# divortio/divortio-lz4

Measured on AMD Instinct MI355X. Metric: LZ4 compress+decompress GB/s on 4 MiB independent blocks; % of HBM peak, higher is better.
Workload: dtype u8; 1 GPU; raw block decompress, 4096 x 4 MiB independent blocks per GPU (tiles216), device-resident (BASELINE.json configs[1]); blocks_per_gpu=4096, block_bytes=4194304, generator=tiles216, parallelism=blocks sharded x1

## Files before the change

divortio-lz4_amd/csrc/lz4mi_decompress.hip:

```cpp
#include "../../include/lz4mi.h"
#include "lz4mi_common.h"
#include "lz4mi_decompress.h"
#include "lz4mi_launch.h"

#ifndef LZ4MI_LL_ADAPT
#define LZ4MI_LL_ADAPT 127
#endif
#ifndef LZ4MI_ORDER
#define LZ4MI_ORDER 1
#endif
#ifndef LZ4MI_ABLATE
#define LZ4MI_ABLATE 0
#endif

#ifndef LZ4MI_TIMELINE
#define LZ4MI_TIMELINE 0
#endif

#ifndef LZ4MI_PROFILE
#define LZ4MI_PROFILE 0
#endif

namespace lz4mi {

// ... 639 lines not shown
            }
            P += lane_of(incl, kWave - 1);
            R += (uint32_t)__popcll(bal);
        }
        __syncthreads();
        PieceGen g{L, bm, P, 0u, -1, lane};
        while (64u * g.t < P) {
            LSlot sl[kPieceBatch];
            uint4 v[kPieceBatch];
            g.template fill<kPieceBatch>(sl);
#pragma unroll
            for (int j = 0; j < kPieceBatch; ++j) {
                const u32x4_t t = *(const u32x4_t*)(c.dst + (sl[j].w ? sl[j].a : 0));
                v[j] = make_uint4(t.x, t.y, t.z, t.w);
            }
            lane_store<kPieceBatch>(c, S, sl, v);
        }
        __syncthreads();
    }
}

__device__ __forceinline__ void lane_slow_run(const Ctx& c, const DecShared& S, const Run& R) {
    const int np = run_pieces(R.n);
    for (int p = 0; p < np; ++p) {
        const Piece P = plan_piece(R, p);
        if (P.mode == 4) {
            bytes_piece(c, P.y, P.a, P.b, P.w, P.period);
            continue;
        }
        const uint4 A = load16<R_HIST>(c, S, P.a);
        uint4 v = A;
        if (P.mode == 2) v = pick4(A, load16<R_HIST>(c, S, P.b), P.k);
        else if (P.mode == 3) v = expand_period(A, P.k, P.period);
        store_w(c.dst + P.y, v, P.w);
    }
}

__device__ __forceinline__ void periodic_run(const Ctx& c, const DecShared& S, int lane, const Run& R, PatBuf B) {
    const int32_t per = R.period;
    const uint8_t* src = c.dst + R.src;
    const int32_t W = B.bytes - 48;
    const int32_t dl = R.n - 16;
    for (int32_t s0 = 0; s0 < per; s0 += W) {
        const int32_t e0 = per - s0 <= W ? per : s0 + W;
        __syncthreads();
        for (int k = lane; 16 * k < e0 - s0 + 20; k += kWave) {
            const int32_t q = s0 + 16 * k;
            uint4 v;
            if (q + 16 <= per) {
                v = load16<R_HIST>(c, S, R.src + q);
            } else {
                unsigned __int128 x = 0;
#pragma unroll 1
                for (int j = 0; j < 16; ++j) x |= (unsigned __int128)src[(q + j) % per] << (8 * j);
                __builtin_memcpy(&v, &x, 16);
            }
            B.w[4 * k] = v.x;
            B.w[4 * k + 1] = v.y;
            B.w[4 * k + 2] = v.z;
            B.w[4 * k + 3] = v.w;
        }
        __syncthreads();
        const int32_t a0 = (int32_t)((0u - (uint32_t)(uintptr_t)(c.dst + R.y)) & 15u);
        if (lane == 0 && a0) {
            const int32_t ph = 0 - s0;
            if ((uint32_t)ph < (uint32_t)(e0 - s0)) out16(c.dst + R.y, stage16(B.w, ph));
        }
        const int32_t np = (R.n - a0 + 15) >> 4;
        const int32_t step = (16 * kWave) % per;
        int32_t r = (a0 + 16 * lane) % per;
#pragma unroll 2
        for (int32_t p = lane; p < np; p += kWave) {
            const int32_t d0 = a0 + 16 * p;
            const bool last = d0 > dl;
            const int32_t d = last ? dl : d0;
            const int32_t ph = (last ? d % per : r) - s0;
            if ((uint32_t)ph < (uint32_t)(e0 - s0) && LZ4MI_ABLATE != 4) {
                out16(c.dst + R.y + d, stage16(B.w, ph));
            }
            r += step;
            if (r >= per) r -= per;
        }
    }
    __syncthreads();
}


__device__ __forceinline__ void long_literals(uint8_t* dst, const uint8_t* src, int32_t n, int lane) {
    const int32_t np = (n + 15) >> 4;
    auto at = [&](int32_t p) { return 16 * p < n - 16 ? 16 * p : n - 16; };
#if LZ4MI_LL_ADAPT
    const unsigned int* lat = &g_lat_active[32 * xcc_id()];
#endif
    for (int32_t p0 = lane; p0 < np; p0 += kWave * 4) {
#if LZ4MI_LL_ADAPT
        const uint32_t busy = __hip_atomic_load(lat, __ATOMIC_RELAXED, __HIP_MEMORY_SCOPE_AGENT);
#endif
        const int32_t d0 = at(p0), d1 = at(p0 + kWave), d2 = at(p0 + 2 * kWave), d3 = at(p0 + 3 * kWave);
        uint4 v0, v1, v2, v3;
        v0 = ld16_nt(src + d0);
        v1 = ld16_nt(src + d1);
        v2 = ld16_nt(src + d2);
        v3 = ld16_nt(src + d3);
        st16_nt(dst + d0, v0);
        st16_nt(dst + d1, v1);
        st16_nt(dst + d2, v2);
        st16_nt(dst + d3, v3);
#if LZ4MI_LL_ADAPT
        if (busy) __builtin_amdgcn_s_sleep(LZ4MI_LL_ADAPT);
#endif
    }
}

__device__ __forceinline__ void wave_run(const Ctx& c, DecShared& S, int lane, const Run& R, PatBuf B) {
    if (R.kind == R_NONE || R.n <= 0) return;
    const bool in_buf = R.kind == R_HIST || (R.kind == R_BYTES && c.out_off + R.src >= 0);
    if (in_buf && R.period && R.n > kPeriodBulk &&
        B.bytes > 0 && (R.period + 48 <= B.bytes || (R.n >= 4 * R.period && B.bytes >= 1024))) {
        periodic_run(c, S, lane, R, B);
        return;
    }
    const int np = run_pieces(R.n);
    if (R.kind == R_BYTES) {
        for (int p = lane; p < np; p += kWave) {
            const Piece P = plan_piece(R, p);
            bytes_piece(c, P.y, P.a, P.b, P.w, P.period);
        }
        return;
    }
    if (R.period) {
        WaveGen<kWaveB2> g{R, np, 0, lane};
        pipe<R_HIST, true, kWaveB2>(c, S, g);
        return;
    }
    WaveGen<kWaveB> g{R, np, 0, lane};
    if (R.kind == R_LDS) pipe<R_LDS, false, kWaveB>(c, S, g);
    else if (R.kind == R_COMP && R.n >= kLongLit) long_literals(c.dst + R.y, c.blk + R.src, R.n, lane);
    else if (R.kind == R_COMP) pipe<R_COMP, false, kWaveB>(c, S, g);
    else pipe<R_HIST, false, kWaveB>(c, S, g);
}

__device__ __forceinline__ void short_literals(const Ctx& c, int32_t y, int32_t n, const uint4& v) {
    if (LZ4MI_ABLATE == 4) return;
    uint8_t* d = c.dst + y;
    uint64_t lo = v.x | ((uint64_t)v.y << 32);
    const uint64_t hi = v.z | ((uint64_t)v.w << 32);
    int32_t o = 0;
    if (n & 8) { __builtin_memcpy(d, &lo, 8); lo = hi; o = 8; }
    if (n & 4) { const uint32_t t = (uint32_t)lo; __builtin_memcpy(d + o, &t, 4); lo >>= 32; o += 4; }
    if (n & 2) { const uint16_t t = (uint16_t)lo; __builtin_memcpy(d + o, &t, 2); lo >>= 16; o += 2; }
    if (n & 1) d[o] = (uint8_t)lo;
}

__device__ __forceinline__ void lane_literals(const Ctx& c, const DecShared& S, const Run& L) {
    const int32_t n = L.kind == R_NONE ? 0 : L.n;
    const int np = n >= 16 ? (n + 15) >> 4 : 0;
    for (int q = 0; __ballot(q < np) != 0; q += 2) {
        const int32_t d0 = 16 * q < n - 16 ? 16 * q : n - 16, d1 = 16 * (q + 1) < n - 16 ? 16 * (q + 1) : n - 16;
        const uint4 v0 = stage16(S.stage, L.src + d0);
        const uint4 v1 = stage16(S.stage, L.src + d1);
        if (LZ4MI_ABLATE == 4) continue;
        if (q < np) out16(c.dst + L.y + d0, v0);
        if (q + 1 < np) out16(c.dst + L.y + d1, v1);
    }
    if (__ballot(n > 0 && n < 16)) {
        if (n > 0 && n < 16) short_literals(c, L.y, n, stage16(S.stage, L.src));
    }
}

__device__ __forceinline__ int64_t wave_varint(const Ctx& c, int lane, int64_t& q) {
    int64_t sum = 0;
    for (;;) {
        int64_t p = q + 16 * lane;
        int first = 16;
        uint32_t lastb = 0;
        for (int j = 0; j < 16; ++j) {
            int64_t r = p + j;
            uint32_t b = (r < c.in_len) ? c.blk[r] : 0u;
            if (b != 255u && first == 16) { first = j; lastb = b; }
        }
        uint64_t mask = __ballot(first < 16);
        if (mask) {
            int fl = __builtin_ctzll(mask);
            int fi = lane_of(first, fl);
            uint32_t fb = lane_of(lastb, fl);
            int64_t cnt = (int64_t)fl * 16 + fi;
            sum += 255 * cnt + fb;
            q += cnt + 1;
            return sum;
        }
        sum += 255 * 16 * kWave;
        q += 16 * kWave;
    }
}

__device__ __forceinline__ uint32_t seq_error(const Ctx& c, int64_t out_start, int64_t lit, int64_t ll, uint32_t off,
                                              int64_t ml) {
    if (out_start + ll > c.cap) return 1;
    if (lit + ll > c.in_len) return 2;
    if (ml == 0) return 0;
    if (off == 0) return 3;
    int64_t ms_abs = c.out_off + out_start + ll;
    if ((int64_t)off > ms_abs + c.dict_len) return 4;
    if (c.isolate && (int64_t)off > out_start + ll) return 5;
    return 0;
}

__device__ __forceinline__ int32_t err_status(uint32_t e) { return e == 5 ? -9 : -(int32_t)e; }
template <bool XP>
__device__ __forceinline__ uint32_t seq_err(const Ctx& c, bool rel, int64_t out_start, int64_t lit, int64_t ll,
                                            uint32_t off, int64_t ml) {
    if (XP && rel) {
        if (lit + ll > c.in_len) return 2;
        if (ml == 0) return 0;
        return off == 0 ? 3u : 0u;
    }
    return seq_error(c, out_start, lit, ll, off, ml);
}

__device__ __forceinline__ uint32_t f1_changes(const Ctx& c, int32_t ms, int32_t off, int32_t ml) {
    if (ml == 0 || ml >= 8 || off < 8 || c.out_off + ms - off < 0) return 0;
    const int32_t p0 = ms + ml - 8;
    if (p0 - off < 0) return c.isolate ? 2u : 1u;
    for (int32_t p = p0; p < ms && p < c.cap; ++p)
        if (hist_u8(c.dst + p) != hist_u8(c.dst + p - off)) return 1;
    return 0;
}

__device__ __noinline__ void f1_fixup(const Ctx c, const DecShared& S, int lane, uint32_t nseq, bool cut, int64_t cut_ms,
                         int32_t coff, int32_t cml) {
    int64_t lo = INT64_MAX;
    const uint32_t n = nseq + (cut ? 1u : 0u);
    for (uint32_t k = 0; k < n; ++k) {
        int64_t ms;
        int32_t off, ml;
        if (k < nseq) {
            const SeqInfo q = seq_info(S, k);
            ms = (int64_t)q.out + q.ll;
            off = q.off;
            ml = q.ml;
        } else {
            ms = cut_ms;
            off = coff;
            ml = cml;
        }
        if (ml == 0) continue;
        const bool internal = c.out_off + ms - off >= 0;
        if (ms - off + ml > lo) {
            if (internal) {
                for (int32_t t = lane; t < ml; t += kWave) {
                    const int64_t d = ms + t;
                    const int64_t s = ms - off + (off < ml ? t % off : t);
                    const uint32_t v = hist_u8(c.dst + s);
                    if (d < c.cap) c.dst[d] = (uint8_t)v;
                }
            } else if (lane == 0) {
                for (int32_t t = 0; t < ml; ++t) {
                    const uint32_t v = hist_byte(c, ms - off + t);
                    if (ms + t < c.cap) c.dst[ms + t] = (uint8_t)v;
                }
            }
            wait_vmem();
        }
        if (internal && off >= 8 && ml < 8) {
            const int64_t p = ms + ml - 8 + lane;
            const bool mine = lane < 8 - ml && c.out_off + p >= 0 && p < c.cap;
            const uint32_t v = mine ? (c.out_off + p - off >= 0 ? hist_u8(c.dst + p - off) : 0u) : 0u;
            if (mine) c.dst[p] = (uint8_t)v;
            const int64_t p0 = ms + ml - 8;
            if (p0 < lo) lo = p0;
            wait_vmem();
        }
    }
}

__device__ __forceinline__ void stored_block(const DecArgs& a, const Ctx& c, uint32_t b, uint32_t out_cap, int lane) {
    int32_t status = 0;
    const int32_t n = c.in_len;
    if ((uint32_t)n > out_cap) {
        status = LZ4MI_ERR_RANGE_STATUS;
    } else if (n >= 16) {
        long_literals(c.dst, c.blk, n, lane);
    } else if (lane < n) {
        c.dst[lane] = c.blk[lane];
    }
    if (lane == 0) {
        a.status[b] = status;
        a.out_len[b] = status ? 0u : (uint32_t)n;
    }
}

struct XState {
    bool on = false;
    uint4* xs = nullptr;
    SegRec* xr = nullptr;
    uint32_t seg_lo = 0, seg_hi = 0;
    bool started = false, done = false, fail = false;
    uint32_t G = 0, X = 0, nx = 0, olen = 0, err = 0xFFFFFFFFu, entry = 0;
    int64_t OG = 0;
    int pass = 0, restart = 0;
};

template <bool LK>
__device__ __forceinline__ bool x_enter(const DecArgs& a, Ctx& c, XState& x, int lane, uint32_t wblk, uint32_t sg,
                                        uint32_t nseg, uint32_t out_cap) {
    x.on = LK || ((uint32_t)c.in_len <= a.x_in_max && out_cap <= a.x_out_max &&
                  (uint64_t)out_cap < (uint64_t)c.in_len * kXRatioMax &&
                  !(a.x_flat1 && (uint64_t)c.in_len * 16 >= (uint64_t)out_cap * 15));
    if (!x.on) return a.xphase == 0 && sg == wblk % nseg;
    const SegGeom G = seg_geom((uint32_t)c.in_len);
    if (sg >= G.S) return false;
    x.seg_lo = sg * G.L;
    x.seg_hi = sg + 1 == G.S ? (uint32_t)c.in_len : min((uint32_t)c.in_len, x.seg_lo + G.L);
    x.xs = a.xseq + (size_t)wblk * a.xseq_stride + (size_t)sg * G.stride;
    x.xr = a.xrec + (size_t)wblk * nseg + sg;
    SegRec* const xr = x.xr;
    if (a.xphase == 2) {
        const uint32_t from = uniform(xr->from);
        if (from == kNoBase) return false;
        x.pass = 2;
        x.entry = from;
    }
    if (a.xphase == 1) {
        const uint32_t sstar = a.xfirst[wblk];
        if (sg < sstar) return false;
        uint32_t fp = 0;
        if (sg == sstar) {
            fp = xr[-1].exit;
        } else {
            if (lane == 0) {
                const uint32_t* f = &xr[-1].fin;
                while ((fp = __hip_atomic_load(f, __ATOMIC_ACQUIRE, __HIP_MEMORY_SCOPE_AGENT)) == 0u)
                    __builtin_amdgcn_s_sleep(8);
            }
            fp = lane_of(fp, 0) - 1u;
        }
        uint32_t fin = 0;
        bool reparse = false;
        if (fp == kFinErr) {
            fin = kFinErr;
            if (lane == 0) { xr->cnt = 0; xr->olen = 0; xr->err = 0xFFFFFFFFu; }
        } else if (fp >= x.seg_hi) {
            fin = fp;
            if (lane == 0) { xr->entry = xr->exit = fp; xr->cnt = 0; xr->olen = 0; xr->err = 0xFFFFFFFFu; }
        } else if (sg != sstar && !xr->fail && xr->entry == fp) {
            fin = xr->err != 0xFFFFFFFFu ? kFinErr : xr->exit;
        } else {
            reparse = true;
        }
        if (!reparse) {
            if (lane == 0) __hip_atomic_store(&xr->fin, fin + 1u, __ATOMIC_RELEASE, __HIP_MEMORY_SCOPE_AGENT);
            return false;
        }
        x.pass = 1;
        x.entry = fp;
    }
    c.ip = x.pass ? (int32_t)x.entry
                  : (x.seg_lo >= (uint32_t)c.in_len ? c.in_len : (int32_t)(x.seg_lo - min(x.seg_lo, kSegWarm)));
    return true;
}

__device__ __forceinline__ void stage_loads(const Ctx& c, int64_t at, int lane, uint4& p0, uint4& p1) {
    p0 = stage_piece(c, at + 16 * opaque(lane));
    if (lane < kStageWords / 4 - kWave) p1 = stage_piece(c, at + 16 * (kWave + opaque(lane)));
}
__device__ __forceinline__ void stage_write(DecShared& S, int lane, const uint4& p0, const uint4& p1) {
    __builtin_memcpy((uint8_t*)S.stage + 16 * lane, &p0, 16);
    if (lane < kStageWords / 4 - kWave) __builtin_memcpy((uint8_t*)S.stage + 16 * (kWave + lane), &p1, 16);
}

struct Prefetch {
    uint4 pf0 = make_uint4(0, 0, 0, 0), pf1 = make_uint4(0, 0, 0, 0);
    int64_t pf_at = -1;
    bool have_pf = false;
};
__device__ __forceinline__ void prefetch(const Ctx& c, Prefetch& pf, int64_t at, int lane) {
    stage_loads(c, at, lane, pf.pf0, pf.pf1);
    pf.pf_at = at;
    pf.have_pf = true;
}
__device__ __forceinline__ void settle(Prefetch& pf) {
    settle(pf.pf0);
    settle(pf.pf1);
}

__device__ __forceinline__ void stage_chunk(const Ctx& c, DecShared& S, Prefetch& pf, int lane) {
    if (!pf.have_pf || pf.pf_at != c.ip) {
        uint4 p0, p1 = make_uint4(0, 0, 0, 0);
        stage_loads(c, (int64_t)c.ip, lane, p0, p1);
        stage_write(S, lane, p0, p1);
    } else {
        stage_write(S, lane, pf.pf0, pf.pf1);
    }
    pf.have_pf = false;
    __syncthreads();
}

struct Parse {
    uint32_t vis, tail, last_tok;
    int last_lane;
    bool cut;
};
__device__ __forceinline__ Parse parse_chunk(DecShared& S, int lane, uint32_t rem, bool fast_tab, Prof& prof) {
    const uint8_t* s = (const uint8_t*)S.stage;
    const uint32_t seg0 = 16u * lane, seg1 = seg0 + 16;
    uint32_t vis, tail;
    PROF(0);
    __builtin_amdgcn_s_setprio(0);
    uint16_t* nxt = S.nxt;
    if (fast_tab) {
        next_table_fast(S.stage, nxt, lane);
    } else {
        static_assert(kChunk % kWave == 0, "whole rows per lane");
        uint32_t slm = 0;
#pragma unroll
        for (int i = 0; i < kChunk / kWave; ++i) {
            bool slow;
            const uint32_t v = next_fast(s, lane + kWave * i, rem, slow);
            slm |= (slow ? 1u : 0u) << i;
            nxt[lane + kWave * i] = enc_next(v);
        }
        if (__ballot(slm != 0)) {
            for (uint32_t m = slm; m; m &= m - 1) {
                const uint32_t p = lane + kWave * __builtin_ctz(m);
                nxt[p] = enc_next(next_token(s, p, rem));
            }
        }
    }
    __syncthreads();
    jump_table(nxt, S.nxt2, lane);
    __syncthreads();
    jump_table(S.nxt2, S.nxt4, lane);
    __syncthreads();
#if LZ4MI_ABLATE == 3
    return Parse{0u, (uint32_t)kChunk, 0u, 0, false};
#endif

    PROF(1);
    __builtin_amdgcn_s_setprio(1);
    uint32_t x;
    vis = 0;
    {
        uint32_t p = seg0 < kWarm ? 0u : seg0 - kWarm;
        for (uint32_t q; (q = S.nxt4[p]) < seg0;) p = q;
        for (uint32_t q; (q = S.nxt2[p]) < seg0;) p = q;
        while (p < seg1) {
            if (p >= seg0) vis |= 1u << (p - seg0);
            p = next_of(nxt, p);
            PROF_COUNT(15, 1);
        }
        x = p;
    }
    uint32_t es = vis ? seg0 + __builtin_ctz(vis) : x;
    uint32_t nE = 0;
    for (int it = 0; it <= kWave; ++it) {
        const uint32_t pes = dpp<kWaveShr1>(0u, es), px = dpp<kWaveShr1>(0u, x);
        nE = lane == 0 ? 0u : (pes >= seg0 ? pes : px);
        bool valid = nE >= seg1 ? (vis == 0 && x == nE) : ((vis >> (nE - seg0)) & 1u) != 0;
        uint64_t bad = __ballot(!valid);
        PROF_COUNT(13, 1);
        if (it == 0) PROF_COUNT(14, __popcll(bad));
        if (bad == 0) break;
        if (lane == __builtin_ctzll(bad)) {
            vis = 0;
            uint32_t p = nE;
            while (p < seg1) {
                vis |= 1u << (p - seg0);
                p = next_of(nxt, p);
            }
            x = p;
            es = vis ? seg0 + __builtin_ctz(vis) : x;
        }
    }
    if (nE >= seg1) vis = 0;
    else vis &= ~((1u << (nE - seg0)) - 1u);
    tail = lane_of(x, kWave - 1);
    if (tail > (uint32_t)kLim && tail < kEnd) tail = kStop;
    const uint64_t has = __ballot(vis != 0);
    const int last_lane = 63 - __builtin_clzll(has);
    const uint32_t last_tok = lane_val(seg0 + 31 - __builtin_clz(vis | 1u), (uint32_t)last_lane);
    return Parse{vis, tail, last_tok, last_lane, tail == kStop};
}

struct SeqTable {
    uint32_t nseq;
    int64_t total;
    uint32_t first_err;
    bool redo;
};
template <bool XP>
__device__ __forceinline__ SeqTable seq_table(const Ctx& c, DecShared& S, int lane, uint32_t rem, bool rel,
                                              bool fast_tab, const Parse& P, Prof& prof) {
    PROF(2);
    const uint8_t* s = (const uint8_t*)S.stage;
    const uint32_t seg0 = 16u * lane;
    const uint32_t cnt = __popc(P.vis) - ((P.cut && lane == P.last_lane) ? 1u : 0u);
    const uint32_t incl = wave_incl_scan(cnt, lane);
    const uint32_t base = incl - cnt;
    const uint32_t nseq = lane_of(incl, kWave - 1);
    uint16_t* const tl = (uint16_t*)S.pms;
    static_assert(sizeof(uint16_t) * (kMaxSeq + 2 * kWave) <= sizeof(S.pms), "token list fits in the pending starts");
    {
        uint32_t m = P.vis;
        for (uint32_t j = 0; j < cnt; ++j) {
            tl[base + j] = (uint16_t)(seg0 + __builtin_ctz(m));
            m &= m - 1;
        }
    }
    __syncthreads();
    const bool exact_all = !rel && c.O > (int64_t)c.cap;
    const uint32_t capr = rel || exact_all ? 0xFFFFFFFFu : (uint32_t)(c.cap - (int32_t)c.O);
    const int64_t d4 = c.out_off + c.dict_len;
    const uint32_t L45 = rel || exact_all ? 0x80000000u
                                          : (uint32_t)c.O + (c.isolate ? 0u : (uint32_t)(d4 < 65536 ? d4 : 65536));
    uint32_t carry = 0;
    uint32_t first_err = 0xFFFFFFFFu;
    uint32_t flagged = 0xFFFFFFFFu;
    constexpr int kRows = 2;
    for (uint32_t i0 = 0; i0 < nseq; i0 += kRows * kWave) {
        uint32_t p[kRows], tok[kRows], b1[kRows];
#pragma unroll
        for (int r = 0; r < kRows; ++r) {
            const uint32_t k = i0 + kWave * r + lane;
            p[r] = k < nseq ? tl[k] : 0u;
        }
#pragma unroll
        for (int r = 0; r < kRows; ++r) {
            tok[r] = s[p[r]];
            b1[r] = s[p[r] + 1];
        }
        uint32_t q[kRows], lit[kRows], ll[kRows], o0[kRows], o1[kRows], mb[kRows];
#pragma unroll
        for (int r = 0; r < kRows; ++r) {
            const uint32_t x1 = (tok[r] >> 4) == 15 ? 1u : 0u;
            ll[r] = x1 ? 15u + b1[r] : tok[r] >> 4;
            lit[r] = p[r] + 1 + x1;
            q[r] = lit[r] + ll[r];
            const uint32_t qa = q[r] + 2 <= (uint32_t)kLim ? q[r] : 0u;
            o0[r] = s[qa];
            o1[r] = s[qa + 1];
            mb[r] = s[qa + 2];
        }
        uint32_t off[kRows], ml[kRows];
        bool rerun = false;
#pragma unroll
        for (int r = 0; r < kRows; ++r) {
            const bool live = i0 + kWave * r + lane < nseq;
            off[r] = 0;
            ml[r] = 0;
            if (!live) {
                ll[r] = 0;
                continue;
            }
            uint32_t qj = q[r];
            if ((tok[r] >> 4) == 15 && b1[r] == 255) {
                uint32_t t = p[r] + 1, bb, llj = 15;
                do { bb = s[t++]; llj += bb; } while (bb == 255);
                ll[r] = llj;
                lit[r] = t;
                qj = t + llj;
                if (qj < rem) { o0[r] = s[qj]; o1[r] = s[qj + 1]; mb[r] = s[qj + 2]; }
            }
            if (qj < rem) {
                off[r] = o0[r] | (o1[r] << 8);
                uint32_t m = tok[r] & 15;
                if (m == 15) {
                    if (mb[r] != 255) {
                        m += mb[r];
                    } else {
                        rerun |= fast_tab;
                        uint32_t t = qj + 2, bb;
                        do { bb = s[t++]; m += bb; } while (bb == 255 && t < (uint32_t)kLim);
                    }
                }
                ml[r] = m + 4;
            }
        }
        if (__ballot(rerun)) return SeqTable{0u, 0, 0xFFFFFFFFu, true};
        bool flag = false;
#pragma unroll
        for (int r = 0; r < kRows; ++r) {
            if (r > 0 && i0 + kWave * r >= nseq) break;
            const uint32_t k = i0 + kWave * r + lane;
            const uint32_t len = ll[r] + ml[r];
            const uint32_t sc = wave_incl_scan(len, lane);
            const uint32_t ro = carry + sc - len;
            carry += lane63(sc);
            if (k < nseq) {
                S.t_seq[k] = make_uint4((uint32_t)c.O + ro, lit[r] | (ll[r] << 16), off[r] | (ml[r] << 16), 0u);
                const uint32_t X = ro + ll[r];
                flag |= X > capr || lit[r] + ll[r] > rem || (ml[r] != 0 && off[r] - 1u >= L45 + X);
            }
        }
        if (__ballot(flag) != 0 && flagged > i0) flagged = i0;
    }
    __syncthreads();
    for (uint32_t i0 = exact_all ? 0u : flagged; i0 < nseq && first_err == 0xFFFFFFFFu; i0 += kWave) {
        const uint32_t k = i0 + lane;
        uint32_t e = 0;
        if (k < nseq) {
            const SeqInfo q = seq_info(S, k);
            e = seq_err<XP>(c, rel, c.O + (uint32_t)(q.out - (int32_t)c.O), (int64_t)c.ip + q.lit, q.ll, q.off, q.ml);
        }
        first_err = wave_min(e ? (k << 3) | e : 0xFFFFFFFFu);
    }
    return SeqTable{nseq, (int64_t)carry, first_err, false};
}

struct CutSeq {
    int64_t cq = 0, cll = 0, cml = 0, clit = 0;
    uint32_t coff = 0;
};

__device__ __forceinline__ void advance(Ctx& c, int64_t tab_hi, const Parse& P, const CutSeq& cs) {
    c.O = tab_hi;
    if (P.cut) {
        c.O += cs.cll + cs.cml;
        c.ip = (int32_t)(cs.cq < c.in_len ? cs.cq : c.in_len);
    } else if (P.tail >= kEnd) {
        c.ip = c.in_len;
    } else {
        c.ip += (int32_t)P.tail;
    }
}

__device__ __forceinline__ void x_export_chunk(Ctx& c, const DecShared& S, XState& x, int lane, const Parse& P,
                                               const SeqTable& T, const CutSeq& cs) {
    const bool cut = P.cut;
    const uint32_t nseq = T.nseq, seg_lo = x.seg_lo, seg_hi = x.seg_hi;
    const int64_t tab_hi = c.O + T.total;
    const uint32_t ipc = (uint32_t)c.ip;
    const uint32_t ntot = nseq + (cut ? 1u : 0u);
    const uint32_t ecut = cut ? seq_err<true>(c, true, tab_hi, cs.clit, cs.cll, cs.coff, cs.cml) : 0u;
    const uint32_t ferr = T.first_err != 0xFFFFFFFFu ? T.first_err : (ecut ? ((nseq << 3) | ecut) : 0xFFFFFFFFu);
    const uint32_t fk = ferr == 0xFFFFFFFFu ? ntot : (ferr >> 3);
    auto x_tok = [&](uint32_t k) -> uint32_t {
        if (k >= nseq) return ipc + P.last_tok;
        const SeqInfo q = seq_info(S, k);
        return ipc + (uint32_t)q.lit - 1u - (q.ll >= 15 ? (uint32_t)(q.ll - 15) / 255u + 1u : 0u);
    };
    auto x_out = [&](uint32_t k) -> int64_t { return k >= nseq ? tab_hi : (int64_t)S.t_seq[k].x; };
    uint32_t k0 = ntot, k1 = ntot;
    for (uint32_t r = 0; 64u * r < ntot; ++r) {
        const uint32_t k = 64u * r + lane;
        const uint32_t t = k < ntot ? x_tok(k) : 0xFFFFFFFFu;
        const uint64_t m0 = __ballot(k < ntot && t >= seg_lo), m1 = __ballot(k < ntot && t >= seg_hi);
        if (k0 == ntot && m0) k0 = 64u * r + (uint32_t)__builtin_ctzll(m0);
        if (k1 == ntot && m1) k1 = 64u * r + (uint32_t)__builtin_ctzll(m1);
    }
    bool restart = false;
    if (!x.started && fk < k0) {
        if (x.pass == 0 && x.restart < kSegRestarts) {
            restart = true;
            ++x.restart;
        } else {
            x.fail = x.done = true;
        }
    } else {
        if (!x.started && k0 < ntot) {
            x.started = true;
            x.G = x_tok(k0);
            x.OG = x_out(k0);
        }
        if (x.started) {
            const uint32_t ke = fk < k1 ? fk + 1 : k1;
            for (uint32_t k = k0 + lane; k < ke; k += kWave) {
                uint4 e;
                if (k < nseq) {
                    const SeqInfo q = seq_info(S, k);
                    e = make_uint4((uint32_t)(x_out(k) - x.OG), ipc + (uint32_t)q.lit, (uint32_t)q.ll,
                                   q.ml ? (uint32_t)q.off : 0u);
                } else {
                    e = make_uint4((uint32_t)(tab_hi - x.OG), (uint32_t)cs.clit, (uint32_t)cs.cll,
                                   cs.cml ? cs.coff : 0u);
                }
                x.xs[x.nx + (k - k0)] = e;
            }
            if (fk < k1) {
                x.err = ((x.nx + (fk - k0)) << 3) | (ferr & 7u);
                x.done = true;
            } else if (k1 < ntot) {
                x.done = true;
                x.X = x_tok(k1);
                x.olen = (uint32_t)(x_out(k1) - x.OG);
            }
            x.nx += ke - k0;
        }
    }
    if (restart) {
        c.ip = (int32_t)(x_tok(fk) + 1u);
        c.O = 0;
    } else if (!x.done) {
        advance(c, tab_hi, P, cs);
        if ((uint32_t)c.ip >= seg_hi && c.ip < c.in_len) {
            if (!x.started) {
                x.started = true;
                x.G = (uint32_t)c.ip;
                x.OG = c.O;
            }
            x.done = true;
            x.X = (uint32_t)c.ip;
            x.olen = (uint32_t)(c.O - x.OG);
        }
    }
    __syncthreads();
}

__device__ __forceinline__ void x_finish(const DecArgs& a, const Ctx& c, XState& x, int lane, uint32_t sg) {
    if (!x.done) {
        if (!x.started) {
            x.G = (uint32_t)c.in_len;
            x.OG = c.O;
        }
        x.X = (uint32_t)c.in_len;
        x.olen = (uint32_t)(c.O - x.OG);
    }
    if (lane == 0) {
        SegRec* const xr = x.xr;
        xr->entry = x.G;
        xr->exit = x.X;
        xr->cnt = x.nx;
        xr->olen = x.olen;
        xr->err = x.err;
        xr->fail = (x.fail || (a.xforce && sg > 0 && (a.xforce == 2 ? x.pass != 1 : x.pass == 0))) ? 1u : 0u;
        if (x.pass == 1)
            __hip_atomic_store(&xr->fin, (x.err != 0xFFFFFFFFu ? kFinErr : x.X) + 1u, __ATOMIC_RELEASE,
                               __HIP_MEMORY_SCOPE_AGENT);
    }
}

__device__ __forceinline__ uint32_t source_map(const Ctx& c, DecShared& S, int lane, uint32_t nseq, int64_t total) {
    uint32_t msh = total >= 32u * nseq ? 5u : 4u;
    while ((total >> msh) >= kLim) ++msh;
    for (uint32_t k = lane; k < nseq; k += kWave) {
        const uint32_t t0 = S.t_seq[k].x - (uint32_t)c.O;
        const uint32_t t1 = (k + 1 < nseq ? S.t_seq[k + 1].x : (uint32_t)(c.O + total)) - (uint32_t)c.O;
        for (uint32_t b = (t0 + (1u << msh) - 1) >> msh; (b << msh) < t1; ++b) S.nxt[b] = (uint16_t)k;
    }
    __syncthreads();
    return msh;
}

__device__ __forceinline__ uint32_t round1(const Ctx& c, DecShared& S, int lane, uint32_t nseq, uint32_t msh, Prof& prof) {
    uint32_t pend = 0;
    uint32_t ready = 0;
    uint32_t rbits = 0;
    uint32_t nlit_pack = 0;
    for (uint32_t i = 0; 64 * i < nseq; ++i) {
        const uint32_t k = 64 * i + lane;
        Run M = no_run(), ML = no_run();
        SeqInfo q = seq_info(S, k < nseq ? k : 0u);
        if (k >= nseq) q.ll = 0;
        {
            const Run L = q.ll ? Run{q.out, q.ll, q.lit, 0, R_LDS} : no_run();
            const bool longL = L.n > kLaneBytes;
            lane_literals(c, S, longL ? no_run() : L);
            for (uint64_t lm = __ballot(longL); lm; lm &= lm - 1) wave_run(c, S, lane, shfl_run(L, __builtin_ctzll(lm)), no_pat());
        }
        PROF(23);
        if (k < nseq) {
            const int32_t t0 = q.out;
            M = match_run(c, t0 + q.ll, q.off, q.ml);
            if (M.n == 0) {
                M.kind = R_NONE;
            } else if (match_src_end(M) > (int32_t)c.O) {
                int32_t rs = M.src, re = match_src_end(M), li = 0, nl = 0;
                const int r = (M.kind == R_HIST && M.period == 0)
                                  ? remap_src(c, S, nseq, msh, rs, re, li, nl, i < 4)
                                  : 0;
                if (r == 3) {
                    ML = Run{M.y, nl, li, 0, R_LDS};
                    M.y += nl;
                    M.n -= nl;
                    nlit_pack |= (uint32_t)nl << (8 * i);
                }
                if (r == 1 || r == 3) {
                    M.src = rs;
                    if (c.out_off + rs < 16) M.kind = R_BYTES;
                    S.t_seq[k].w = (uint32_t)(rs + (r == 3 ? kSplitBase : kMemoBase));
                    rbits |= 1u << i;
                } else if (r == 2) {
                    ML = Run{M.y, M.n, li, 0, R_LDS};
                    M.kind = R_NONE;
                } else {
                    pend |= 1u << i;
                    M.kind = R_NONE;
                }
            }
        }
        const bool longM = M.kind != R_NONE && M.n > kLaneBytes;
        const bool longML = ML.n > kLaneBytes;
        const bool fastM = M.kind == R_HIST && M.period == 0 && M.n >= 16;
        if (M.kind != R_NONE && !longM && fastM) ready |= 1u << i;
        PROF(16);
        lane_literals(c, S, longML ? no_run() : ML);
        PROF(17);
        for (uint64_t lm = __ballot(longML); lm; lm &= lm - 1) wave_run(c, S, lane, shfl_run(ML, __builtin_ctzll(lm)), no_pat());
        if (M.kind != R_NONE && !longM && !fastM) lane_slow_run(c, S, M);
        for (uint64_t mm = __ballot(longM); mm; mm &= mm - 1) wave_run(c, S, lane, shfl_run(M, __builtin_ctzll(mm)), pat_round1(S));
        PROF(18);
    }
    piece_pipe(c, S, ready, rbits, lane, nseq, nlit_pack);
    return pend;
}

__device__ __forceinline__ void later_rounds(const Ctx& c, DecShared& S, int lane, uint32_t nseq, uint32_t pend,
                                             Prof& prof) {
    for (; LZ4MI_ABLATE != 6;) {
        uint32_t np = 0;
        for (uint32_t i = 0; 64 * i < nseq; ++i) {
            const bool pk = (pend >> i) & 1u;
            const uint64_t bal = __ballot(pk);
            if (pk) {
                const uint32_t k = 64 * i + lane;
                const uint32_t idx = np + __builtin_amdgcn_mbcnt_hi((uint32_t)(bal >> 32),
                                                                    __builtin_amdgcn_mbcnt_lo((uint32_t)bal, 0u));
                const SeqInfo q = seq_info(S, k);
                const int32_t ms = q.out + q.ll;
                S.pms[idx] = (uint32_t)ms;
                S.pme[idx] = (uint32_t)(ms + q.ml > c.cap ? c.cap : ms + q.ml);
            }
            np += (uint32_t)__popcll(bal);
        }
        if (np == 0) break;
        PROF_COUNT(11, 1);
        __syncthreads();
        wait_vmem();
        PROF(20);
        uint32_t ready = 0;
        for (uint32_t i = 0; 64 * i < nseq; ++i) {
            if (__ballot((pend >> i) & 1u) == 0) continue;
            Run M = no_run();
            if ((pend >> i) & 1u) {
                const uint32_t k = 64 * i + lane;
                const SeqInfo q = seq_info(S, k);
                M = match_run(c, q.out + q.ll, q.off, q.ml);
                const int32_t rs = M.src, re = match_src_end(M);
                uint32_t lo = 0, hi = np;
                while (lo < hi) {
                    const uint32_t mid = (lo + hi) >> 1;
                    if ((int32_t)S.pme[mid] > rs) hi = mid;
                    else lo = mid + 1;
                }
                if (lo >= np || (int32_t)S.pms[lo] >= re) pend &= ~(1u << i);
                else M.kind = R_NONE;
            }
            const bool longM = M.kind != R_NONE && M.n > kLaneBytes;
            const bool fastM = M.kind == R_HIST && M.period == 0 && M.n >= 16;
            if (M.kind != R_NONE && !longM && fastM) ready |= 1u << i;
            if (M.kind != R_NONE && !longM && !fastM) lane_slow_run(c, S, M);
            for (uint64_t mm = __ballot(longM); mm; mm &= mm - 1) wave_run(c, S, lane, shfl_run(M, __builtin_ctzll(mm)), pat_rounds(S));
        }
        piece_pipe(c, S, ready, 0u, lane, nseq, 0u);
        __syncthreads();
    }
}

__device__ __forceinline__ void output_rounds(const Ctx& c, DecShared& S, int lane, const SeqTable& T, Prof& prof) {
    const uint32_t msh = source_map(c, S, lane, T.nseq, T.total);
    PROF(22);
    const uint32_t pend = round1(c, S, lane, T.nseq, msh, prof);
    PROF(19);
    later_rounds(c, S, lane, T.nseq, pend, prof);
}

__device__ __forceinline__ int32_t f1_table(const Ctx& c, const DecShared& S, int lane, uint32_t nseq) {
    bool cand = false;
    for (uint32_t k = lane; k < nseq; k += kWave) {
        const SeqInfo q = seq_info(S, k);
        cand |= q.ml != 0 && q.ml < 8 && q.off >= 8;
    }
    if (__ballot(cand)) {
        wait_vmem();
        uint32_t dv = 0;
        for (uint32_t k = lane; k < nseq; k += kWave) {
            const SeqInfo q = seq_info(S, k);
            dv |= f1_changes(c, q.out + q.ll, q.off, q.ml);
        }
        if (__ballot(dv & 2u)) return -9;
        if (__ballot(dv)) f1_fixup(c, S, lane, nseq, false, 0, 0, 0);
    }
    return 0;
}

__device__ __forceinline__ int32_t cut_match(const Ctx& c, DecShared& S, int lane, int32_t ms, const CutSeq& cs,
                                             bool f1check) {
    const Run M = match_run(c, ms, (int32_t)cs.coff, (int32_t)cs.cml);
    if (M.n > 0) {
        wait_vmem();
        wave_run(c, S, lane, M, pat_all(S));
    }
    if (f1check && cs.cml != 0 && cs.cml < 8 && cs.coff >= 8) {
        wait_vmem();
        const uint32_t dv = lane == 0 ? f1_changes(c, ms, (int32_t)cs.coff, (int32_t)cs.cml) : 0u;
        if (__ballot(dv & 2u)) return -9;
        if (__ballot(dv)) f1_fixup(c, S, lane, 0, true, (int64_t)ms, (int32_t)cs.coff, (int32_t)cs.cml);
    }
    return 0;
}

constexpr bool kOutput = LZ4MI_ABLATE == 0 || LZ4MI_ABLATE >= 4;
constexpr bool kParseOnly = LZ4MI_ABLATE == 2 || LZ4MI_ABLATE == 3;

template <bool XP, bool LK = false>
__device__ __forceinline__ void decompress_block(const DecArgs& a) {
    __shared__ DecShared S;
    const int lane = threadIdx.x;
    const uint32_t nseg = XP ? a.xsegs : 1u;
    if (blockIdx.x >= a.nblocks * nseg) return;
    const uint32_t wblk = XP ? blockIdx.x / nseg : blockIdx.x;
    const uint32_t sg = XP ? blockIdx.x - wblk * nseg : 0u;
    if (LK && uniform(a.xcnt[wblk]) == kNotExported) return;
    const uint32_t b = a.order ? uniform(a.order[wblk]) : wblk;
    if (!XP && a.redo && !uniform(a.redo[b])) return;
#if LZ4MI_TIMELINE
    const uint64_t tl_t0 = wall_clock64();
#endif
    const uint64_t in_off = uniform64(a.in_off[b]), out_off = uniform64(a.out_off[b]);
    const uint32_t out_cap = uniform(a.out_cap[b]);
    Ctx c;
    c.blk = a.in + in_off;
    const uint32_t word = uniform(a.in_len[b]);
    c.in_len = (int32_t)(a.frame_words ? word & 0x7FFFFFFFu : word);
    c.out_off = (int64_t)out_off;
    c.dst = a.out + out_off;
    c.cap = out_cap > 0x7FFFFFFFu ? 0x7FFFFFFF : (int32_t)out_cap;
    c.dict = a.dict;
    c.dict_len = a.dict ? (int32_t)a.dict_len : 0;
    c.isolate = a.isolate;
    c.ip = 0;
    c.O = 0;
    if (a.frame_words && (word & 0x80000000u)) {
        stored_block(a, c, b, out_cap, lane);
        return;
    }
    XState x;
    if constexpr (XP) {
        if (!x_enter<LK>(a, c, x, lane, wblk, sg, nseg, out_cap)) return;
    }
    const bool xp = XP && x.on;
#if LZ4MI_LL_ADAPT
    const bool lat_bound = (uint64_t)c.in_len * 2 < (uint64_t)out_cap;
    unsigned int* lat = &g_lat_active[32 * xcc_id()];
    if (lat_bound && lane == 0) atomicAdd(lat, 1u);
#endif
    Prefetch pf;
    Prof prof;
#if LZ4MI_PROFILE
    prof = Prof{{0}, (uint64_t)wall_clock64()};
#endif
    int32_t status = 0;
    while (c.ip < c.in_len) {
        if (XP && x.done) break;
        PROF_COUNT(10, 1);
        stage_chunk(c, S, pf, lane);
        const uint32_t rem = (uint32_t)(c.in_len - c.ip);
        Parse P;
        SeqTable T;
        for (bool fast_tab = rem > kFastRem;; fast_tab = false) {
            P = parse_chunk(S, lane, rem, fast_tab, prof);
            if (LZ4MI_ABLATE != 3 && !P.cut && P.tail < kEnd && (int64_t)c.ip + P.tail < c.in_len)
                prefetch(c, pf, (int64_t)c.ip + P.tail, lane);
            if (kParseOnly) break;
            T = seq_table<XP>(c, S, lane, rem, xp, fast_tab, P, prof);
            if (!T.redo) break;
            wait_vmem();
            settle(pf);
            __syncthreads();
        }
        if (kParseOnly) {
            c.ip = P.tail == kEnd ? c.in_len : c.ip + (P.cut ? kChunk : (int32_t)P.tail);
            __syncthreads();
            continue;
        }
        if (T.first_err != 0xFFFFFFFFu && !xp) { status = err_status(T.first_err & 7); break; }
        PROF(3);
        CutSeq cs;
        {
            const uint8_t* s = (const uint8_t*)S.stage;
            int64_t cq = 0, cll = 0, cml = 0, clit = 0;
            uint32_t coff = 0;
            if (P.cut) {
                constexpr uint32_t kStaged = 16 * (kStageWords / 4);
                uint32_t r = P.last_tok;
                const uint32_t tok = s[r++];
                cll = tok >> 4;
                bool more = cll == 15;
                while (more && r < kStaged) {
                    const uint32_t b = s[r++];
                    cll += b;
                    more = b == 255;
                }
                int64_t q = (int64_t)c.ip + r;
                if (more) cll += wave_varint(c, lane, q);
                clit = q;
                q += cll;
                if (q < c.in_len) {
                    uint32_t w[4];
                    if (q + 16 <= c.in_len) {
                        __builtin_memcpy(w, c.blk + q, 16);
                    } else {
                        const uint4 t = load16_tail(c.blk, q, c.in_len);
                        w[0] = t.x;
                        w[1] = t.y;
                        w[2] = t.z;
                        w[3] = t.w;
                    }
                    coff = w[0] & 0xFFFFu;
                    q += 2;
                    cml = tok & 15;
                    if (cml == 15) {
                        bool run = true;
                        for (int t = 2; t < 16 && run; ++t) {
                            const uint32_t wd = t < 4 ? w[0] : t < 8 ? w[1] : t < 12 ? w[2] : w[3];
                            const uint32_t b = (wd >> (8 * (t & 3))) & 255u;
                            cml += b;
                            ++q;
                            run = b == 255;
                        }
                        if (run) cml += wave_varint(c, lane, q);
                    }
                    cml += 4;
                }
                cq = q;
            }
            cs = CutSeq{cq, cll, cml, clit, coff};
        }
        if constexpr (XP) {
            if (xp) {
                x_export_chunk(c, S, x, lane, P, T, cs);
                continue;
            }
        }
        const int64_t tab_hi = c.O + T.total;
        if (P.cut && cs.cq < c.in_len) prefetch(c, pf, cs.cq, lane);
        if (kOutput) {
            PROF(4);
            __builtin_amdgcn_s_setprio(3);
            wait_vmem();
            settle(pf);
            PROF(21);
            output_rounds(c, S, lane, T, prof);
            PROF(6);
        }
        if (P.cut) {
            if (kOutput) PROF_COUNT(12, 1);
            const uint32_t e = seq_error(c, tab_hi, cs.clit, cs.cll, cs.coff, cs.cml);
            if (e) { status = err_status(e); break; }
            if (kOutput)
                wave_run(c, S, lane, Run{(int32_t)tab_hi, (int32_t)cs.cll, (int32_t)cs.clit, 0, cs.cll ? (uint32_t)R_COMP : (uint32_t)R_NONE}, no_pat());
        }
        PROF(7);
        if (a.f1check) {
            status = f1_table(c, S, lane, T.nseq);
            if (status) break;
        }
        if (kOutput && P.cut) {
            status = cut_match(c, S, lane, (int32_t)(tab_hi + cs.cll), cs, a.f1check);
            if (status) break;
        }
        advance(c, tab_hi, P, cs);
        __syncthreads();
        PROF(8);
    }
    if constexpr (XP) {
        if (xp) {
            x_finish(a, c, x, lane, sg);
#if LZ4MI_LL_ADAPT
            if (lat_bound && lane == 0) atomicSub(lat, 1u);
#endif
            return;
        }
    }
#if LZ4MI_PROFILE
    if (lane == 0)
        for (int i = 0; i < 24; ++i) atomicAdd(&g_prof[i], (unsigned long long)prof.acc[i]);
#endif
    if (lane == 0) {
        a.status[b] = status;
        a.out_len[b] = status ? 0u : (uint32_t)c.O;
        if (XP) a.xcnt[b] = kNotExported;
    }
#if LZ4MI_LL_ADAPT
    if (lat_bound && lane == 0) atomicSub(lat, 1u);
#endif
#if LZ4MI_TIMELINE
    wait_vmem();
    const uint64_t tl_t1 = wall_clock64();
    uint32_t hw, xcc;
    asm volatile("s_getreg_b32 %0, hwreg(HW_REG_HW_ID)" : "=s"(hw));
    asm volatile("s_getreg_b32 %0, hwreg(HW_REG_XCC_ID)" : "=s"(xcc));
    if (lane == 0 && b < kTlMax) {
        g_tl[2 * b] = tl_t0;
        g_tl[2 * b + 1] = tl_t1;
        g_tl_id[2 * b] = hw;
        g_tl_id[2 * b + 1] = xcc;
    }
#endif
}

__global__ __launch_bounds__(64, 4) void lz4mi_decompress_kernel(DecArgs a) { decompress_block<false>(a); }
__global__ __launch_bounds__(64, 4) void lz4mi_decompress_x_kernel(DecArgs a) { decompress_block<true>(a); }
__global__ __launch_bounds__(64, 4) void lz4mi_decompress_xl_kernel(DecArgs a) { decompress_block<true, true>(a); }

__global__ __launch_bounds__(64) void lz4mi_xverify_kernel(DecArgs a) {
    static_assert(kSegMax == 4 * 64, "four records per lane");
    const uint32_t b = blockIdx.x, lane = threadIdx.x;
    if (a.xcnt[b] == kNotExported) return;
    const uint32_t nseg = a.xsegs, in_len = a.in_len[b];
    const SegGeom G = seg_geom(in_len);
    SegRec* R = a.xrec + (size_t)b * nseg;
    uint32_t entry[4], exit[4], err[4], fail[4], hi_l[4], my_fin[4], kind[4];
#pragma unroll
// ... 248 lines not shown
```

Baseline: 1484 GB/s.

## Deal literal copies across lanes in 16-byte pieces and defer cut sequences

Replaces per-lane literal copying with a wave-wide work list. Every literal run of at least 16 bytes is recorded in shared memory along with a bitmap of piece starts, and the 16-byte pieces are then spread evenly over all lanes, so one long run no longer leaves the other lanes idle. Long-literal wave runs are folded into the same dealt list. Separately, when a chunk is cut mid-sequence, parsing now stops at the last token so the next chunk handles it, avoiding the cut-sequence path. In exchange it adds extra syncthreads, LDS atomics and a scan, and reuses the pms buffer, which risks aliasing.

```diff
diff --git a/divortio-lz4_amd/csrc/lz4mi_decompress.hip b/divortio-lz4_amd/csrc/lz4mi_decompress.hip
--- a/divortio-lz4_amd/csrc/lz4mi_decompress.hip
+++ b/divortio-lz4_amd/csrc/lz4mi_decompress.hip
@@ -815,20 +815,74 @@
     if (n & 1) d[o] = (uint8_t)lo;
 }
 
-__device__ __forceinline__ void lane_literals(const Ctx& c, const DecShared& S, const Run& L) {
-    const int32_t n = L.kind == R_NONE ? 0 : L.n;
-    const int np = n >= 16 ? (n + 15) >> 4 : 0;
-    for (int q = 0; __ballot(q < np) != 0; q += 2) {
-        const int32_t d0 = 16 * q < n - 16 ? 16 * q : n - 16, d1 = 16 * (q + 1) < n - 16 ? 16 * (q + 1) : n - 16;
-        const uint4 v0 = stage16(S.stage, L.src + d0);
-        const uint4 v1 = stage16(S.stage, L.src + d1);
-        if (LZ4MI_ABLATE == 4) continue;
-        if (q < np) out16(c.dst + L.y + d0, v0);
-        if (q + 1 < np) out16(c.dst + L.y + d1, v1);
-    }
-    if (__ballot(n > 0 && n < 16)) {
-        if (n > 0 && n < 16) short_literals(c, L.y, n, stage16(S.stage, L.src));
-    }
+constexpr int kLitRuns = 64;
+constexpr int kLitRows = kLitRuns * (kLaneBytes / 16) / 64;
+static_assert((kChunk + 16) / 17 <= kLitRuns, "every run of >= 16 literal bytes of a chunk has a list entry");
+static_assert(kLim / 16 + kLitRuns <= 3 * 64, "a chunk's own runs: at most three piece rows");
+static_assert(kLim / 16 + kLitRuns <= kLitRows * 64, "... which the bitmap holds");
+static_assert(kLitRuns * sizeof(PEnt) + kLitRows * 8 <= sizeof(uint32_t) * kMaxSeq, "run list and bitmap fit S.pms");
+static_assert(kLitRows <= kWave, "one lane clears each bitmap word");
+static_assert(offsetof(DecShared, pms) % 16 == 0, "16-byte aligned list entries");
+
+struct LitDeal {
+    uint32_t P = 0, R = 0;
+    static __device__ __forceinline__ PEnt* list(DecShared& S) { return reinterpret_cast<PEnt*>(S.pms); }
+    static __device__ __forceinline__ uint64_t* bitmap(DecShared& S) {
+        return reinterpret_cast<uint64_t*>(reinterpret_cast<uint8_t*>(S.pms) + kLitRuns * sizeof(PEnt));
+    }
+    __device__ __forceinline__ void add(DecShared& S, int lane, bool has, uint64_t bal, int32_t y, int32_t src, int32_t n) {
+        if (R == 0) {
+            if (lane < kLitRows) bitmap(S)[lane] = 0;
+            __syncthreads();
+        }
+        const uint32_t np = has ? (uint32_t)(n + 15) >> 4 : 0u;
+        const uint32_t incl = wave_incl_scan(np, lane);
+        const uint32_t r = R + __builtin_amdgcn_mbcnt_hi((uint32_t)(bal >> 32), __builtin_amdgcn_mbcnt_lo((uint32_t)bal, 0u));
+        const uint32_t p0 = P + incl - np;
+        if (has) {
+            list(S)[r] = PEnt{y, src, n, (int32_t)p0};
+            atomicOr((unsigned long long*)&bitmap(S)[p0 >> 6], 1ull << (p0 & 63u));
+        }
+        P += lane_of(incl, kWave - 1);
+        R += (uint32_t)__popcll(bal);
+    }
+    __device__ __forceinline__ void flush(const Ctx& c, DecShared& S, int lane) {
+        if (R == 0) return;
+        __syncthreads();
+        const PEnt* L = list(S);
+        const uint64_t* bm = bitmap(S);
+        int32_t rb = -1;
+        for (uint32_t t = 0; 64u * t < P; ++t) {
+            const uint64_t w = bm[t];
+            const int32_t below = (int32_t)__builtin_amdgcn_mbcnt_hi((uint32_t)(w >> 32), __builtin_amdgcn_mbcnt_lo((uint32_t)w, 0u));
+            const int32_t r = rb + below + (int32_t)((w >> lane) & 1u);
+            rb += __popcll(w);
+            const uint32_t p = 64u * t + (uint32_t)lane;
+            if (p < P) {
+                const PEnt e = L[r];
+                const int32_t d0 = 16 * ((int32_t)p - e.p0);
+                const int32_t d = d0 < e.n - 16 ? d0 : e.n - 16;
+                const uint4 v = stage16(S.stage, e.src + d);
+                if (LZ4MI_ABLATE != 4) out16(c.dst + e.y + d, v);
+            }
+        }
+        __syncthreads();
+        P = R = 0;
+    }
+};
+
+__device__ __forceinline__ void dealt_literals(const Ctx& c, DecShared& S, int lane, uint32_t nseq) {
+    LitDeal D;
+    for (uint32_t i = 0; 64 * i < nseq; ++i) {
+        const uint32_t k = 64 * i + lane;
+        const uint4& e = S.t_seq[k < nseq ? k : 0u];
+        const uint32_t y = e.x, lw = e.y;
+        const uint32_t n = k < nseq ? lw >> 16 : 0u;
+        const bool has = n >= 16;
+        const uint64_t bal = __ballot(has);
+        if (bal) D.add(S, lane, has, bal, (int32_t)y, (int32_t)(lw & 0xFFFFu), (int32_t)n);
+    }
+    D.flush(c, S, lane);
 }
 
 __device__ __forceinline__ int64_t wave_varint(const Ctx& c, int lane, int64_t& q) {
@@ -1064,7 +1118,7 @@
     int last_lane;
     bool cut;
 };
-__device__ __forceinline__ Parse parse_chunk(DecShared& S, int lane, uint32_t rem, bool fast_tab, Prof& prof) {
+__device__ __forceinline__ Parse parse_chunk(DecShared& S, int lane, uint32_t rem, bool fast_tab, bool defer, Prof& prof) {
     const uint8_t* s = (const uint8_t*)S.stage;
     const uint32_t seg0 = 16u * lane, seg1 = seg0 + 16;
     uint32_t vis, tail;
@@ -1137,11 +1191,16 @@
     }
     if (nE >= seg1) vis = 0;
     else vis &= ~((1u << (nE - seg0)) - 1u);
-    tail = lane_of(x, kWave - 1);
+    const uint32_t raw = lane_of(x, kWave - 1);
+    tail = raw;
     if (tail > (uint32_t)kLim && tail < kEnd) tail = kStop;
     const uint64_t has = __ballot(vis != 0);
     const int last_lane = 63 - __builtin_clzll(has);
     const uint32_t last_tok = lane_val(seg0 + 31 - __builtin_clz(vis | 1u), (uint32_t)last_lane);
+    if (defer && fast_tab && tail == kStop && raw < kEnd && last_tok != 0 && raw - last_tok <= (uint32_t)kLim) {
+        if (lane == last_lane) vis &= ~(1u << (last_tok - seg0));
+        return Parse{vis, last_tok, last_tok, last_lane, false};
+    }
     return Parse{vis, tail, last_tok, last_lane, tail == kStop};
 }
 
@@ -1409,16 +1468,18 @@
     uint32_t ready = 0;
     uint32_t rbits = 0;
     uint32_t nlit_pack = 0;
+    dealt_literals(c, S, lane, nseq);
+    LitDeal D;
     for (uint32_t i = 0; 64 * i < nseq; ++i) {
         const uint32_t k = 64 * i + lane;
         Run M = no_run(), ML = no_run();
         SeqInfo q = seq_info(S, k < nseq ? k : 0u);
         if (k >= nseq) q.ll = 0;
         {
-            const Run L = q.ll ? Run{q.out, q.ll, q.lit, 0, R_LDS} : no_run();
-            const bool longL = L.n > kLaneBytes;
-            lane_literals(c, S, longL ? no_run() : L);
-            for (uint64_t lm = __ballot(longL); lm; lm &= lm - 1) wave_run(c, S, lane, shfl_run(L, __builtin_ctzll(lm)), no_pat());
+            const bool shortL = q.ll > 0 && q.ll < 16;
+            if (__ballot(shortL)) {
+                if (shortL) short_literals(c, q.out, q.ll, stage16(S.stage, q.lit));
+            }
         }
         PROF(23);
         if (k < nseq) {
@@ -1456,13 +1517,26 @@
         const bool fastM = M.kind == R_HIST && M.period == 0 && M.n >= 16;
         if (M.kind != R_NONE && !longM && fastM) ready |= 1u << i;
         PROF(16);
-        lane_literals(c, S, longML ? no_run() : ML);
+        {
+            const bool dealML = ML.n >= 16 && !longML, shortML = ML.n > 0 && ML.n < 16;
+            if (const uint64_t bal = __ballot(dealML)) {
+                if (D.R + (uint32_t)__popcll(bal) > (uint32_t)kLitRuns) D.flush(c, S, lane);
+                D.add(S, lane, dealML, bal, ML.y, ML.src, ML.n);
+            }
+            if (__ballot(shortML)) {
+                if (shortML) short_literals(c, ML.y, ML.n, stage16(S.stage, ML.src));
+            }
+        }
         PROF(17);
         for (uint64_t lm = __ballot(longML); lm; lm &= lm - 1) wave_run(c, S, lane, shfl_run(ML, __builtin_ctzll(lm)), no_pat());
         if (M.kind != R_NONE && !longM && !fastM) lane_slow_run(c, S, M);
-        for (uint64_t mm = __ballot(longM); mm; mm &= mm - 1) wave_run(c, S, lane, shfl_run(M, __builtin_ctzll(mm)), pat_round1(S));
+        if (const uint64_t mm0 = __ballot(longM)) {
+            D.flush(c, S, lane);
+            for (uint64_t mm = mm0; mm; mm &= mm - 1) wave_run(c, S, lane, shfl_run(M, __builtin_ctzll(mm)), pat_round1(S));
+        }
         PROF(18);
     }
+    D.flush(c, S, lane);
     piece_pipe(c, S, ready, rbits, lane, nseq, nlit_pack);
     return pend;
 }
@@ -1621,7 +1695,7 @@
         Parse P;
         SeqTable T;
         for (bool fast_tab = rem > kFastRem;; fast_tab = false) {
-            P = parse_chunk(S, lane, rem, fast_tab, prof);
+            P = parse_chunk(S, lane, rem, fast_tab, !XP, prof);
             if (LZ4MI_ABLATE != 3 && !P.cut && P.tail < kEnd && (int64_t)c.ip + P.tail < c.in_len)
                 prefetch(c, pf, (int64_t)c.ip + P.tail, lane);
             if (kParseOnly) break;
```

After: 1618 GB/s, median of 6. +9.0%, better.
